# TravisWheelerLab/BATH

Measured on AMD Instinct MI355X. Metric: DP Gcells/s + residues/s through bathsearch pipeline at 1/2/4/8 MI355X, higher is better.
Workload: dtype u8/i16 integer scores (SSV: exact binary16), f32 Forward

## Files before the change

### bath_amd/csrc/bath_profile.hip

```cpp
#include <atomic>
#include <cctype>
#include <cmath>
#include <cstring>

#include "bath_common.hpp"
#include "host_model.hpp"

using namespace bath;

namespace bath {

static const double kLog2 = 0.69314718055994529;

double gumbel_surv(double x, double mu, double lambda) {
  double ey = -std::exp(-lambda * (x - mu));
  if (std::fabs(ey) < 5e-9) return -ey;
  return 1.0 - std::exp(ey);
}
double gumbel_invsurv(double p, double mu, double lambda) {
  double lp = (p < 5e-9) ? (std::pow(p, p) - 1) / p : std::log(-1. * std::log(1 - p));
  return mu - lp / lambda;
}
double exp_surv(double x, double mu, double lambda) { return (x < mu) ? 1.0 : std::exp(-lambda * (x - mu)); }

static inline uint8_t cost_u8(float scale, float sc) {
  float c = -1.0f * roundf(scale * sc);
  return (c > 255.) ? 255 : (uint8_t)(int)c;
}
static inline uint8_t cost_u8_biased(float scale, uint8_t bias, float sc) {
  float c = -1.0f * roundf(scale * sc);
  return (c > 255 - bias) ? 255 : (uint8_t)((int)c + bias);
}
static inline int16_t score_i16(float scale, float sc) {
  float v = roundf(scale * sc);
  if (v >= 32767.0) return 32767;
  if (v <= -32768.0) return -32768;
  return (int16_t)v;
}

void bias_filter_eo(const float *compo, float eo[kKp][2]) {
  for (int x = 0; x < 20; x++) { eo[x][0] = kAminoBg[x] / kAminoBg[x]; eo[x][1] = compo[x] / kAminoBg[x]; }
  for (int x : {20, 27, 28}) eo[x][0] = eo[x][1] = 1.0f;
  for (int x = 21; x <= 26; x++)
    for (int s = 0; s < 2; s++) {
      float num = 0.f, den = 0.f;
      for (int y = 0; y < 20; y++)
        if (amino_degen_has(x, y)) { num += (s == 0 ? kAminoBg[y] : compo[y]); den += kAminoBg[y]; }
      eo[x][s] = den > 0.f ? num / den : 0.f;
    }
}

template <class T>
static hipError_t upload(T **dst, const T *src, size_t n, hipStream_t st) {
  hipError_t e = hipMalloc((void **)dst, n * sizeof(T) + 64);
  if (e != hipSuccess) return e;
  return hipMemcpyAsync(*dst, src, n * sizeof(T), hipMemcpyHostToDevice, st);
}

int build_len_tables(const bath_hip_oprofile *om, int maxL) {
  std::lock_guard<std::mutex> lock(om->grow_mu);
  LenTables &lt = om->lt;
  if (maxL <= lt.maxL) return BATH_OK;
  bath_hip_ctx *ctx = om->ctx;
  int n = std::max(maxL, 4096) + 1;
  for (void *p : {(void *)lt.d_tjb, (void *)lt.d_xwmove, (void *)lt.d_pmove, (void *)lt.d_nullsc, (void *)lt.d_lt1, (void *)lt.d_lt2, (void *)lt.d_p1})
    if (p) om->retired.push_back(p);
  lt.d_tjb = nullptr; lt.d_xwmove = nullptr; lt.d_pmove = nullptr; lt.d_nullsc = nullptr; lt.d_lt1 = nullptr; lt.d_lt2 = nullptr; lt.d_p1 = nullptr;
  lt.h_tjb.resize(n); lt.h_xwmove.resize(n); lt.h_pmove.resize(n); lt.h_nullsc.resize(n);
  std::vector<float> lt1(n), lt2(n), p1v(n);
  for (int L = 0; L < n; L++) {
    lt.h_tjb[L] = cost_u8(om->scale_b, logf(3.0f / (float)(L + 3)));
    float pmove = (2.0f + om->nj) / ((float)L + 2.0f + om->nj);
    lt.h_pmove[L] = pmove;
    lt.h_xwmove[L] = score_i16(om->scale_w, logf(pmove));
    float p1 = (float)L / (float)(L + 1);
    p1v[L] = p1;
    lt.h_nullsc[L] = (float)((float)L * std::log((double)p1) + std::log(1. - p1));
    lt1[L] = (float)L * logf(p1);
    lt2[L] = logf((float)(1. - p1));
  }
  BATH_HIP_TRY(ctx, upload(&lt.d_tjb, lt.h_tjb.data(), n, ctx->stream));
  BATH_HIP_TRY(ctx, upload(&lt.d_xwmove, lt.h_xwmove.data(), n, ctx->stream));
  BATH_HIP_TRY(ctx, upload(&lt.d_pmove, lt.h_pmove.data(), n, ctx->stream));
  BATH_HIP_TRY(ctx, upload(&lt.d_nullsc, lt.h_nullsc.data(), n, ctx->stream));
  BATH_HIP_TRY(ctx, upload(&lt.d_lt1, lt1.data(), n, ctx->stream));
  BATH_HIP_TRY(ctx, upload(&lt.d_lt2, lt2.data(), n, ctx->stream));
  BATH_HIP_TRY(ctx, upload(&lt.d_p1, p1v.data(), n, ctx->stream));
  BATH_HIP_TRY(ctx, hipStreamSynchronize(ctx->stream));
  lt.maxL = n - 1;
  return BATH_OK;
}

}

int bath_hip_oprofile::ensure_len_tables(int maxL) const { return bath::build_len_tables(this, maxL); }


namespace bath { std::atomic<int> g_ctx_total{0}, g_ctx_internal{0}; }

extern "C" int bath_hip_init(int device, bath_hip_ctx **out) {
  *out = nullptr;
  int ndev = 0;
  if (hipGetDeviceCount(&ndev) != hipSuccess || ndev <= 0) return BATH_ENODEVICE;
  if (device < 0 || device >= ndev) return BATH_EINVAL;
  bath_hip_ctx *ctx = new bath_hip_ctx();
  ctx->device = device;
  if (const char *e = std::getenv("BATH_HIP_SYNC")) {
    static const bool once = [&] {
      (void)hipSetDevice(device);
      const unsigned fl = (e[0] == 'b') ? hipDeviceScheduleBlockingSync : (e[0] == 'y') ? hipDeviceScheduleYield : hipDeviceScheduleSpin;
      if (hipSetDeviceFlags(fl) != hipSuccess) (void)hipGetLastError();
      return true;
    }();
    (void)once;
  }
  if (hipSetDevice(device) != hipSuccess || hipGetDeviceProperties(&ctx->prop, device) != hipSuccess ||
      hipStreamCreateWithFlags(&ctx->stream, hipStreamNonBlocking) != hipSuccess) {
    delete ctx;
    return BATH_ENODEVICE;
  }
  bath::g_ctx_total.fetch_add(1);
  *out = ctx;
  return BATH_OK;
}

extern "C" void bath_hip_finalize(bath_hip_ctx *ctx) {
  if (!ctx) return;
  bath::g_ctx_total.fetch_sub(1);
  if (ctx->internal) bath::g_ctx_internal.fetch_sub(1);
  (void)hipSetDevice(ctx->device);
  (void)hipStreamSynchronize(ctx->stream);
  delete ctx->lane_pool; ctx->lane_pool = nullptr;
  for (bath_hip_ctx *lane : ctx->lanes) bath_hip_finalize(lane);
  ctx->lanes.clear();
  if (ctx->ev_lanes) (void)hipEventDestroy(ctx->ev_lanes);
  if (ctx->tail_stream) (void)hipStreamDestroy(ctx->tail_stream);
  if (ctx->aux) { bath_hip_finalize(ctx->aux); ctx->aux = nullptr; }
  if (ctx->aux2) { bath_hip_finalize(ctx->aux2); ctx->aux2 = nullptr; }
  if (ctx->aux3) { bath_hip_finalize(ctx->aux3); ctx->aux3 = nullptr; }
  for (auto &b : ctx->scratch) b.release();
  for (auto &b : ctx->pinned) b.release();
  for (auto &b : ctx->stage) b.release();
  ctx->results_pinned.release();
  for (auto e : ctx->ev_pool) (void)hipEventDestroy(e);
  for (auto e : ctx->span_events) (void)hipEventDestroy(e);
  if (ctx->ev_fork) (void)hipEventDestroy(ctx->ev_fork);
  if (ctx->ev_join) (void)hipEventDestroy(ctx->ev_join);
  if (ctx->copy_stream) (void)hipStreamDestroy(ctx->copy_stream);
  if (ctx->side_stream) (void)hipStreamDestroy(ctx->side_stream);
  (void)hipStreamDestroy(ctx->stream);
  delete ctx;
}

extern "C" int bath_hip_trim(bath_hip_ctx *ctx) {
  if (!ctx) return BATH_EINVAL;
  BATH_HIP_TRY(ctx, hipSetDevice(ctx->device));
  BATH_HIP_TRY(ctx, hipStreamSynchronize(ctx->stream));
  delete ctx->lane_pool; ctx->lane_pool = nullptr;
// ... 56 lines not shown
  if (!ctx) return BATH_EINVAL;
  ctx->fs_odds = on ? 1 : 0;
  for (bath_hip_ctx *l : ctx->lanes) l->fs_odds = ctx->fs_odds;
  return BATH_OK;
}

extern "C" int bath_hip_set_fs5_odds(bath_hip_ctx *ctx, int on) {
  if (!ctx) return BATH_EINVAL;
  ctx->fs5_odds = on ? 1 : 0;
  for (bath_hip_ctx *l : ctx->lanes) l->fs5_odds = ctx->fs5_odds;
  return BATH_OK;
}


extern "C" void bath_hip_oprofile_destroy(bath_hip_oprofile *om) {
  if (!om) return;
  for (void *p : {(void *)om->d_emit, (void *)om->d_ssv, (void *)om->d_msv, (void *)om->d_rb, (void *)om->d_rw, (void *)om->d_tw, (void *)om->d_rf, (void *)om->d_tf,
                  (void *)om->d_bias_eo, (void *)om->d_vit_rw, (void *)om->d_vit_tw2, (void *)om->d_vit_rank, (void *)om->lt.d_tjb, (void *)om->lt.d_xwmove, (void *)om->lt.d_pmove,
                  (void *)om->lt.d_nullsc, (void *)om->lt.d_lt1, (void *)om->lt.d_lt2, (void *)om->lt.d_p1, (void *)om->d_cons, (void *)om->d_msc, (void *)om->d_tsc, (void *)om->d_rfb, (void *)om->d_tfb})
    if (p) (void)hipFree(p);
  for (void *p : om->retired) (void)hipFree(p);
  delete om;
}

extern "C" int bath_hip_oprofile_set_consensus(bath_hip_oprofile *om, const char *consensus) {
  if (!om || !consensus) return BATH_EINVAL;
  bath_hip_ctx *ctx = om->ctx;
  static const char syms[] = "ACDEFGHIKLMNPQRSTVWY-BJZOUX*~";
  om->consensus.assign((size_t)om->M + 2, ' ');
  om->cons_digital.assign((size_t)om->M + 1, 255);
  for (int k = 1; k <= om->M && consensus[k]; k++) {
    om->consensus[(size_t)k] = consensus[k];
    const char *q = std::strchr(syms, std::toupper((unsigned char)consensus[k]));
    if (q) om->cons_digital[(size_t)k] = (uint8_t)(q - syms);
  }
  if (!om->d_cons) BATH_HIP_TRY(ctx, hipMalloc(&om->d_cons, (size_t)om->M + 1));
  BATH_HIP_TRY(ctx, hipMemcpy(om->d_cons, om->cons_digital.data(), (size_t)om->M + 1, hipMemcpyHostToDevice));
  return BATH_OK;
}

extern "C" int bath_hip_oprofile_M(const bath_hip_oprofile *om) { return om->M; }

extern "C" int bath_hip_oprofile_convert(bath_hip_ctx *ctx, const bath_profile *gm, bath_hip_oprofile **ret) {
  *ret = nullptr;
  const int M = gm->M;
  if (M < 1) { ctx->set_error("profile has no nodes"); return BATH_EINVAL; }
  const size_t W = (size_t)M + 1;
  auto msc = [&](int k, int x) { return gm->rsc[(size_t)x * W * 2 + 2 * k]; };
  auto tsc = [&](int k, int s) { return gm->tsc[(size_t)k * 8 + s]; };
  enum { MM, IM, DM, BM, MD, DD, MI, II };

  bath_hip_oprofile *om = new bath_hip_oprofile();
  { static std::atomic<uint64_t> next_uid{1}; om->uid = next_uid.fetch_add(1); }
  om->ctx = ctx; om->M = M; om->max_length = gm->max_length; om->nj = gm->nj; om->L0 = gm->L;
  std::memcpy(om->evparam, gm->evparam, sizeof om->evparam);
  std::memcpy(om->compo, gm->compo, sizeof om->compo);

  float maxsc = 0.0f;
  for (int x = 0; x < 20; x++)
    for (size_t i = 0; i < W * 2; i++) maxsc = std::max(maxsc, gm->rsc[(size_t)x * W * 2 + i]);
  om->scale_b = (float)(3.0 / kLog2);
  om->base_b = 190;
  om->bias_b = cost_u8(om->scale_b, (float)(-1.0 * maxsc));
  om->rb.assign((size_t)kKp * W, 255);
  for (int x = 0; x < kKp; x++)
    for (int k = 1; k <= M; k++) om->rb[x * W + k] = cost_u8_biased(om->scale_b, om->bias_b, msc(k, x));
  om->tbm_b = cost_u8(om->scale_b, logf(2.0f / ((float)M * (float)(M + 1))));
  om->tec_b = cost_u8(om->scale_b, logf(0.5f));

  om->scale_w = (float)(500.0 / kLog2);
  om->base_w = 12000;
  om->rw.assign((size_t)kKp * W, -32768);
  for (int x = 0; x < kKp; x++)
    for (int k = 1; k <= M; k++) om->rw[x * W + k] = score_i16(om->scale_w, msc(k, x));
  om->tw.assign(W * 8, -32768);
  for (int k = 1; k <= M; k++) {
    int16_t *t = &om->tw[(size_t)k * 8];
    for (int s : {BM, MM, IM, DM}) t[s] = std::min<int16_t>(score_i16(om->scale_w, tsc(k - 1, s)), 0);
    for (int s : {MD, MI}) t[s] = (k < M) ? std::min<int16_t>(score_i16(om->scale_w, tsc(k, s)), 0) : (int16_t)-32768;
    t[II] = (k < M) ? std::min<int16_t>(score_i16(om->scale_w, tsc(k, II)), -1) : (int16_t)-32768;
    t[DD] = (k < M) ? score_i16(om->scale_w, tsc(k, DD)) : (int16_t)-32768;
  }
  om->xw_E[0] = score_i16(om->scale_w, gm->xsc[0][0]);
  om->xw_E[1] = score_i16(om->scale_w, gm->xsc[0][1]);
  int ddb = -32768;
  for (int k = 2; k < M - 1; k++)
    ddb = std::max(ddb, (int)score_i16(om->scale_w, tsc(k, DD)) + (int)score_i16(om->scale_w, tsc(k + 1, DM)) -
                            (int)score_i16(om->scale_w, tsc(k + 1, BM)));
  om->ddbound_w = (int16_t)ddb;

  om->rf.assign((size_t)kKp * W, 0.f);
  for (int x = 0; x < kKp; x++)
    for (int k = 1; k <= M; k++) om->rf[x * W + k] = expf(msc(k, x));
  om->tf.assign(W * 8, 0.f);
  for (int k = 1; k <= M; k++) {
    float *t = &om->tf[(size_t)k * 8];
    for (int s : {BM, MM, IM, DM}) t[s] = expf(tsc(k - 1, s));
    for (int s : {MD, MI, II, DD}) t[s] = (k < M) ? expf(tsc(k, s)) : 0.f;
  }
  om->xf_E[0] = expf(gm->xsc[0][0]);
  om->xf_E[1] = expf(gm->xsc[0][1]);

  {
    std::vector<float> &pre = om->prefix_lengths, &suf = om->suffix_lengths;
    pre.assign(W, 0.f); suf.assign(W, 0.f);
    float total = 0;
    for (int k = 1; k < M; k++) {
      const float t_mi = om->tf[(size_t)k * 8 + MI], t_ii = om->tf[(size_t)k * 8 + II];
      pre[k] = (t_mi == 0) ? 1.f : (float)(1 + (int)(std::log(1e-7 / t_mi) / std::log((double)t_ii)));
      total += pre[k];
    }
    pre[0] = pre[M] = 0;
    for (int k = 1; k < M; k++) pre[k] /= total;
    suf[M] = pre[M - 1];
    for (int k = M - 1; k >= 1; k--) suf[k] = suf[k + 1] + pre[k - 1];
    for (int k = 2; k < M; k++) pre[k] += pre[k - 1];
  }

  static const bool wide = [] { const char *e = std::getenv("BATH_HIP_SSV_WIDE"); return e && e[0] == '1'; }();
  static const int g2max = [] { const char *e = std::getenv("BATH_HIP_SSV_G2_MAX"); return e ? std::atoi(e) : 304; }();
  int G = (!wide && M > 152 && M <= g2max) ? 2 : 1;
  while (G < 8 && M > 416 * G) G *= 2;
  if (M > 416 * G) { ctx->set_error("model longer than 3328 nodes"); delete om; return BATH_EINVAL; }
  int NR = ((M + G - 1) / G + 1) / 2;
  if (G == 1 && NR <= 112) NR = (NR + 3) / 4 * 4;
  else if (G == 2 && NR <= 76) NR = NR <= 40 ? 40 : (NR <= 72 ? (NR + 7) / 8 * 8 : 76);
  else NR = std::max((NR + 15) / 16 * 16, G > 1 ? 112 : 16);
  NR = std::max(NR, 16);
  om->NR = NR; om->G = G;
  om->ssv_row_bytes = 16 * ((NR * G / 4 + 1) | 1);
  {
    size_t rowsz = (size_t)om->ssv_row_bytes / 2;
    auto half_bits = [](float v) { const _Float16 h = (_Float16)v; int16_t b; std::memcpy(&b, &h, 2); return b; };
    std::vector<int16_t> tab((size_t)kSsvRows * rowsz, half_bits(-1.0f));
    for (int x = 0; x < kKp; x++)
      for (int k = 1; k <= M; k++) {
        const int g = (k - 1) / (2 * NR), q = (k - 1) - g * 2 * NR;
        const int cost = std::min((int)om->rb[x * W + k] - (int)om->bias_b, 127);
        tab[x * rowsz + (size_t)g * 2 * NR + 2 * (q % NR) + q / NR] = half_bits(-(float)cost / 2048.0f);
      }
    BATH_HIP_TRY(ctx, upload(&om->d_ssv, tab.data(), tab.size(), ctx->stream));
    if (G == 1 && NR <= 76) {
      std::vector<int16_t> mtab((size_t)kSsvRows * rowsz, half_bits(-1.0f));
      for (int x = 0; x < kKp; x++)
        for (int k = 1; k <= M; k++) {
          const int q = k - 1;
          const int inc = (int)om->bias_b - (int)om->rb[x * W + k];
          mtab[x * rowsz + 2 * (q % NR) + q / NR] = half_bits((float)inc / 2048.0f);
        }
      BATH_HIP_TRY(ctx, upload(&om->d_msv, mtab.data(), mtab.size(), ctx->stream));
    }
  }
  {
    int NRv = ((M + 1) / 2 + 15) / 16 * 16;
    if (NRv == 80) NRv = std::max(68, ((M + 1) / 2 + 3) / 4 * 4);
    if (NRv <= 112) {
      om->vit_NR = NRv;
      om->vit_rw_pitch = 4 * NRv + 16;
      const size_t rowsz = (size_t)om->vit_rw_pitch / 2;
      std::vector<int16_t> rwt((size_t)30 * rowsz, (int16_t)-32768);
      auto slot = [&](int node) { return node <= NRv ? 2 * (node - 1) : 2 * (node - NRv - 1) + 1; };
      for (int x = 0; x < kKp; x++)
        for (int k = 1; k <= M; k++) rwt[x * rowsz + slot(k)] = om->rw[x * W + k];
      std::vector<uint32_t> tw2((size_t)NRv * 8);
      std::vector<int16_t> rank((size_t)2 * NRv, (int16_t)32767);
      const int Q8 = std::max(2, ((M - 1) / 8) + 1);
      auto twv = [&](int node, int s) -> int { return node <= M ? (int)om->tw[(size_t)node * 8 + s] : -32768; };
      for (int r = 0; r < NRv; r++)
        for (int s = 0; s < 8; s++) tw2[(size_t)r * 8 + s] = ((uint32_t)(uint16_t)twv(r + 1, s)) | ((uint32_t)(uint16_t)twv(NRv + r + 1, s) << 16);
      for (int node = 1; node <= M; node++) rank[(size_t)slot(node)] = (int16_t)(((node - 1) % Q8) * 8 + (node - 1) / Q8);
      BATH_HIP_TRY(ctx, upload(&om->d_vit_rw, rwt.data(), rwt.size(), ctx->stream));
      BATH_HIP_TRY(ctx, upload(&om->d_vit_tw2, tw2.data(), tw2.size(), ctx->stream));
      BATH_HIP_TRY(ctx, upload(&om->d_vit_rank, rank.data(), rank.size(), ctx->stream));
    }
  }
  om->rb_stride = (int)W;
  BATH_HIP_TRY(ctx, upload(&om->d_rb, om->rb.data(), om->rb.size(), ctx->stream));
  BATH_HIP_TRY(ctx, upload(&om->d_rw, om->rw.data(), om->rw.size(), ctx->stream));
  BATH_HIP_TRY(ctx, upload(&om->d_tw, om->tw.data(), om->tw.size(), ctx->stream));
  BATH_HIP_TRY(ctx, upload(&om->d_rf, om->rf.data(), om->rf.size(), ctx->stream));
  BATH_HIP_TRY(ctx, upload(&om->d_tf, om->tf.data(), om->tf.size(), ctx->stream));
  {
    std::vector<float> tfb((size_t)(M + 2) * 8, 0.f), rfb((size_t)kKp * (M + 2), 0.f);
    std::memcpy(tfb.data(), om->tf.data(), sizeof(float) * (size_t)(M + 1) * 8);
    for (int x = 0; x < kKp; x++) std::memcpy(&rfb[(size_t)x * (M + 2)], &om->rf[(size_t)x * W], sizeof(float) * W);
    BATH_HIP_TRY(ctx, upload(&om->d_tfb, tfb.data(), tfb.size(), ctx->stream));
    BATH_HIP_TRY(ctx, upload(&om->d_rfb, rfb.data(), rfb.size(), ctx->stream));
    BATH_HIP_TRY(ctx, hipStreamSynchronize(ctx->stream));
  }
  {
    std::vector<float> lm((size_t)kKp * W, -INFINITY);
    for (int x = 0; x < kKp; x++)
      for (int k = 1; k <= M; k++) lm[(size_t)x * W + k] = msc(k, x);
    BATH_HIP_TRY(ctx, upload(&om->d_msc, lm.data(), lm.size(), ctx->stream));
    BATH_HIP_TRY(ctx, upload(&om->d_tsc, gm->tsc, (size_t)M * 8, ctx->stream));
    BATH_HIP_TRY(ctx, hipStreamSynchronize(ctx->stream));
  }
  {
    float eo[kKp][2];
    bias_filter_eo(om->compo, eo);
    BATH_HIP_TRY(ctx, upload(&om->d_bias_eo, &eo[0][0], (size_t)kKp * 2, ctx->stream));
  }
  BATH_HIP_TRY(ctx, hipStreamSynchronize(ctx->stream));
  int st = om->ensure_len_tables(4096);
  if (st != BATH_OK) { bath_hip_oprofile_destroy(om); return st; }
  *ret = om;
  return BATH_OK;
}

extern "C" int bath_hip_oprofile_scalars(const bath_hip_oprofile *om, int L, bath_oprofile_scalars *o) {
  int st = om->ensure_len_tables(L);
  if (st != BATH_OK) return st;
  o->tbm_b = om->tbm_b; o->tec_b = om->tec_b; o->tjb_b = om->lt.h_tjb[L]; o->base_b = om->base_b; o->bias_b = om->bias_b;
  o->scale_b = om->scale_b;
  o->xw[0][0] = om->xw_E[0]; o->xw[0][1] = om->xw_E[1];
  for (int s = 1; s < 4; s++) { o->xw[s][0] = 0; o->xw[s][1] = om->lt.h_xwmove[L]; }
  o->scale_w = om->scale_w; o->base_w = om->base_w; o->ddbound_w = om->ddbound_w;
  o->xf[0][0] = om->xf_E[0]; o->xf[0][1] = om->xf_E[1];
  for (int s = 1; s < 4; s++) { o->xf[s][1] = om->lt.h_pmove[L]; o->xf[s][0] = 1.0f - om->lt.h_pmove[L]; }
  return BATH_OK;
}

extern "C" int bath_hip_oprofile_get_ssv_scores(const bath_hip_oprofile *om, uint8_t *arr) {
  const size_t W = (size_t)om->M + 1;
  std::memset(arr, 0, W * kKp);
  for (int k = 1; k <= om->M; k++)
    for (int x = 0; x < kKp; x++) arr[(size_t)k * kKp + x] = om->rb[x * W + k];
  return BATH_OK;
}
extern "C" int bath_hip_oprofile_get_vit(const bath_hip_oprofile *om, int16_t *rw, int16_t *tw) {
  std::memcpy(rw, om->rw.data(), om->rw.size() * sizeof(int16_t));
  std::memcpy(tw, om->tw.data(), om->tw.size() * sizeof(int16_t));
  return BATH_OK;
}
extern "C" int bath_hip_oprofile_get_fwd(const bath_hip_oprofile *om, float *rf, float *tf) {
  std::memcpy(rf, om->rf.data(), om->rf.size() * sizeof(float));
  std::memcpy(tf, om->tf.data(), om->tf.size() * sizeof(float));
  return BATH_OK;
}


extern "C" void bath_hip_seqs_destroy(bath_hip_seqs *sq) {
  if (!sq) return;
  for (bath_hip_seqs *part : sq->parts) bath_hip_seqs_destroy(part);
  sq->parts.clear();
  if (sq->is_part) { sq->d_data = nullptr; sq->d_len = nullptr; sq->d_context = nullptr; }
  for (void *p : {(void *)sq->d_data, (void *)sq->d_off, (void *)sq->d_len, (void *)sq->d_context, (void *)sq->d_tile_desc, (void *)sq->d_tile_first,
                  (void *)sq->d_packed, (void *)sq->d_poff, sq->d_exc})
    if (p) (void)hipFree(p);
  if (sq->ev_upload) (void)hipEventDestroy(sq->ev_upload);
  delete sq;
}

extern "C" int64_t bath_hip_seqs_count(const bath_hip_seqs *sq) { return sq->n; }

extern "C" int bath_hip_seqs_set_context(bath_hip_seqs *sq, const int32_t *context) {
  if (!sq || sq->is_part) return BATH_EINVAL;
  bath_hip_ctx *ctx = sq->ctx;
  for (bath_hip_seqs *part : sq->parts) bath_hip_seqs_destroy(part);
  sq->parts.clear();
  sq->cache_minlen = -1;
  if (!context) { if (sq->d_context) (void)hipFree(sq->d_context); sq->d_context = nullptr; sq->h_context.clear(); return BATH_OK; }
  for (int64_t i = 0; i < sq->n; i++) if (context[i] < 0 || context[i] > sq->h_len[(size_t)i]) { ctx->set_error("context longer than its window"); return BATH_EINVAL; }
  sq->h_context.assign(context, context + sq->n);
  if (!sq->d_context) BATH_HIP_TRY(ctx, hipMalloc((void **)&sq->d_context, (size_t)std::max<int64_t>(sq->n, 1) * sizeof(int32_t)));
  if (sq->n > 0) BATH_HIP_TRY(ctx, hipMemcpy(sq->d_context, sq->h_context.data(), (size_t)sq->n * sizeof(int32_t), hipMemcpyHostToDevice));
  return BATH_OK;
}

extern "C" int bath_hip_seqs_create(bath_hip_ctx *ctx, const uint8_t *dsq, const int64_t *offsets, int64_t n, bath_hip_seqs **ret) {
  *ret = nullptr;
  if (n < 0) return BATH_EINVAL;
  bath_hip_seqs *sq = new bath_hip_seqs();
  sq->ctx = ctx; sq->n = n;
  sq->h_off.resize(n); sq->h_len.resize(n);
  int64_t pos = 0;
  bool contiguous_ok = true;
  for (int64_t i = 0; i < n; i++) {
    int64_t L = offsets[i + 1] - offsets[i];
    if (L < 0 || L > INT32_MAX) { delete sq; ctx->set_error("bad sequence offsets"); return BATH_EINVAL; }
    sq->h_off[i] = pos; sq->h_len[i] = (int32_t)L;
    if (pos != offsets[i] - offsets[0]) contiguous_ok = false;
    sq->maxlen = std::max(sq->maxlen, (int32_t)L);
    sq->total += L;
    pos += (L + 15) / 16 * 16;
  }
  sq->total_aligned = pos;
  size_t bytes = (size_t)pos + 64;
  BATH_HIP_TRY(ctx, hipMalloc((void **)&sq->d_data, bytes));
  BATH_HIP_TRY(ctx, hipMalloc((void **)&sq->d_off, (size_t)std::max<int64_t>(n, 1) * sizeof(int64_t)));
  BATH_HIP_TRY(ctx, hipMalloc((void **)&sq->d_len, (size_t)std::max<int64_t>(n, 1) * sizeof(int32_t)));
  BATH_HIP_TRY(ctx, hipMemsetAsync(sq->d_data, 0x1d, bytes, ctx->stream));
  std::vector<uint8_t> staged;
  if (n > 0) {
    if (contiguous_ok) {
      BATH_HIP_TRY(ctx, hipMemcpyAsync(sq->d_data, dsq + offsets[0], (size_t)(offsets[n] - offsets[0]), hipMemcpyHostToDevice, ctx->stream));
    } else {
      staged.assign((size_t)pos, 0x1d);
      for (int64_t i = 0; i < n; i++) std::memcpy(staged.data() + sq->h_off[i], dsq + offsets[i], (size_t)sq->h_len[i]);
      BATH_HIP_TRY(ctx, hipMemcpyAsync(sq->d_data, staged.data(), staged.size(), hipMemcpyHostToDevice, ctx->stream));
    }
    BATH_HIP_TRY(ctx, hipMemcpyAsync(sq->d_off, sq->h_off.data(), (size_t)n * sizeof(int64_t), hipMemcpyHostToDevice, ctx->stream));
    BATH_HIP_TRY(ctx, hipMemcpyAsync(sq->d_len, sq->h_len.data(), (size_t)n * sizeof(int32_t), hipMemcpyHostToDevice, ctx->stream));
  }
  BATH_HIP_TRY(ctx, hipStreamSynchronize(ctx->stream));
  *ret = sq;
  return BATH_OK;
}


namespace {
struct ExcRec { int64_t seq; int32_t pos, code; };

__global__ __launch_bounds__(256) void unpack2_kernel(const uint8_t *__restrict__ packed, const int64_t *__restrict__ poff, const int64_t *__restrict__ off,
                                                      const int32_t *__restrict__ len, uint8_t *__restrict__ data, int64_t n) {
  const int64_t s = (int64_t)blockIdx.x * 4 + (threadIdx.x >> 6);
  if (s >= n) return;
  const int lane = threadIdx.x & 63;
  const int L = len[s];
  const int nb = (L + 3) >> 2;
  const uint8_t *src = packed + poff[s];
  uint8_t *dst = data + off[s];
  const int j_lo = blockIdx.y * 4096, j_hi = min((nb + 3) >> 2, j_lo + 4096);
// ... 97 lines not shown
```

### bath_amd/csrc/bath_viterbi.hip

```cpp
#include <algorithm>

#include "bath_common.hpp"
#include "bath_kernels.hpp"
#include "bath_launch.hpp"

using namespace bath;

namespace bath {

__device__ __forceinline__ s16x2 pk_adds(s16x2 a, s16x2 b) { return __builtin_elementwise_add_sat(a, b); }
__device__ __forceinline__ s16x2 pk_max(s16x2 a, s16x2 b) { return __builtin_elementwise_max(a, b); }
__device__ __forceinline__ s16x2 as_s2(unsigned v) { return __builtin_bit_cast(s16x2, v); }
__device__ __forceinline__ unsigned as_u(s16x2 v) { return __builtin_bit_cast(unsigned, v); }

struct VitLaneTables {
  const int16_t *rw;
  int rw_pitch_bytes;
  const uint32_t *tw2;
  const int16_t *rank;
};

struct VitLaneConsts {
  int M, base_w, xwE_loop, xwE_move, Q8;
  float scale_w;
  double invP_vit, invP_msv;
  float scale_b;
  int base_b, tec_b, bias_b;
};

typedef uint32_t u32x16 __attribute__((ext_vector_type(16)));

template <int NR>
#ifndef BATH_VIT_WAVES
#define BATH_VIT_WAVES 1
#endif
__global__ __launch_bounds__(256, (NR <= 76 ? BATH_VIT_WAVES : 1)) void vit_lane_kernel(SeqView sq, VitLaneTables tb, const uint32_t *__restrict__ tw2g, VitLaneConsts c, const int16_t *__restrict__ xwmove_tab,
                                                          const uint8_t *__restrict__ tjb_tab, const int32_t *__restrict__ todo, int64_t ntodo,
                                                          const int *__restrict__ ntodo_dev, const int *__restrict__ skip_dev, float *__restrict__ sc, int32_t *__restrict__ status,
                                                          const float *__restrict__ filtersc, const uint8_t *__restrict__ ssv_scores,
                                                          WindowRec *__restrict__ wins, int *__restrict__ win_count, int win_cap, int32_t *__restrict__ kminmax) {
  extern __shared__ __attribute__((aligned(16))) char lds[];
  char *s_rw = lds;
  int16_t *s_rank = reinterpret_cast<int16_t *>(lds + 30 * tb.rw_pitch_bytes);
  {
    const uint32_t *src = reinterpret_cast<const uint32_t *>(tb.rw);
    uint32_t *dst = reinterpret_cast<uint32_t *>(s_rw);
    for (int i = threadIdx.x; i < 30 * tb.rw_pitch_bytes / 4; i += blockDim.x) dst[i] = src[i];
    for (int i = threadIdx.x; i < 2 * NR; i += blockDim.x) s_rank[i] = tb.rank[i];
  }
  __syncthreads();
  if (ntodo_dev) ntodo = *ntodo_dev;
  const int64_t t = (int64_t)blockIdx.x * blockDim.x + threadIdx.x + (skip_dev ? *skip_dev : 0);
  if (t - (threadIdx.x & 63) >= ntodo) return;
  const bool live = t < ntodo;
  const int64_t sid = live ? (todo ? (int64_t)todo[t] : t) : (todo ? (int64_t)todo[0] : 0);
  const int L = live ? sq.len[sid] : 0;
  const uint8_t *s = sq.data + sq.off[sid];
  const int Lw = wave_max_i32(L);
  const bool do_win = (wins != nullptr);
  const int M = c.M;

  const int xw_move = xwmove_tab[L];
  int sc_thresh = 0, sc_ext_thresh = 0, skip_until = 0, kmin = 1 << 30, kmax = 0;
  if (do_win && live) {
    const double fsc = (double)filtersc[sid];
    sc_thresh = (int)(int16_t)(int)ceil(((fsc + 0.69314718055994529 * c.invP_vit + 3.0) * (double)c.scale_w) -
                                        (double)(float)c.xwE_move - (double)(float)xw_move + (double)(float)c.base_w);
    sc_ext_thresh = (int)ceil(((fsc + 0.69314718055994529 * c.invP_msv + 3.0) * (double)c.scale_b) + c.base_b + c.tec_b + (int)tjb_tab[L]);
  }
  const s16x2 NEG = {-32768, -32768};
  s16x2 Mr[NR], Ir[NR], Dr[NR];
#pragma unroll
  for (int r = 0; r < NR; r++) Mr[r] = Ir[r] = Dr[r] = NEG;
  int xN = c.base_w;
  int xB = (int16_t)(xN + xw_move);
  int xJ = -32768, xC = -32768;
  bool overflow = false;
  short ePrev = -32768;

  uint32_t wnext = (0 < L) ? *reinterpret_cast<const uint32_t *>(s) : 0x1d1d1d1du;
  for (int i0 = 0; i0 < Lw; i0 += 4) {
    const uint32_t w = wnext;
    wnext = (i0 + 4 < L) ? *reinterpret_cast<const uint32_t *>(s + i0 + 4) : 0x1d1d1d1du;
#pragma unroll 1
    for (int j = 0; j < 4; j++) {
      const int i = i0 + j + 1;
      const bool on = (i <= L) && !overflow;
      int x = (w >> (8 * j)) & 0xff;
      x = (i <= L) ? min(x, kKp - 1) : 29;
      const char *rowbase = s_rw + x * tb.rw_pitch_bytes;
      const s16x2 xBv = {(short)xB, (short)xB};
      s16x2 xEv = NEG;
      unsigned pM = (as_u(Mr[NR - 1]) << 16) | 0x8000u, pI = (as_u(Ir[NR - 1]) << 16) | 0x8000u, pD = (as_u(Dr[NR - 1]) << 16) | 0x8000u;
      s16x2 dpk = NEG;
      s16x2 cpk = {(short)-32768, ePrev};
      int twz = 0;
      asm volatile("" : "+s"(twz));
      const uint32_t *tw = tw2g + twz;
      u32x16 t_c, t_n;
      int4 e_c = *reinterpret_cast<const int4 *>(rowbase), e_n = e_c;
      asm volatile("s_load_dwordx16 %0, %1, 0x0" : "=s"(t_c) : "s"(tw));
#pragma unroll
      for (int r = 0; r < NR; r += 2) {
        asm volatile("s_waitcnt lgkmcnt(0)" ::: "memory");
        __builtin_amdgcn_sched_barrier(0);
        if ((r & 3) == 0 && r + 4 < NR) e_n = *reinterpret_cast<const int4 *>(rowbase + 4 * (r + 4));
        if (r + 2 < NR) asm volatile("s_load_dwordx16 %0, %1, %2" : "=s"(t_n) : "s"(tw), "i"((r + 2) * 32));
        __builtin_amdgcn_sched_barrier(0);
        const unsigned em[2] = {(r & 3) ? (unsigned)e_c.z : (unsigned)e_c.x, (r & 3) ? (unsigned)e_c.w : (unsigned)e_c.y};
#pragma unroll
        for (int q = 0; q < 2; q++) {
          const int rr = r + q;
          const unsigned tMM = t_c[8 * q + 0], tIM = t_c[8 * q + 1], tDM = t_c[8 * q + 2], tBM = t_c[8 * q + 3];
          const unsigned tMD = t_c[8 * q + 4], tDD = t_c[8 * q + 5], tMI = t_c[8 * q + 6], tII = t_c[8 * q + 7];
          const unsigned oM = as_u(Mr[rr]), oI = as_u(Ir[rr]);
          const unsigned oD = as_u(pk_max(Dr[rr], cpk));
          cpk = pk_adds(cpk, as_s2(tDD));
          const s16x2 ms = as_s2(pM), is = as_s2(pI), ds = as_s2(pD);
          s16x2 sv = pk_adds(xBv, as_s2(tBM));
          sv = pk_max(sv, pk_adds(ms, as_s2(tMM)));
          sv = pk_max(sv, pk_adds(is, as_s2(tIM)));
          sv = pk_max(sv, pk_adds(ds, as_s2(tDM)));
          sv = pk_adds(sv, as_s2(em[q]));
          Ir[rr] = pk_max(pk_adds(as_s2(oM), as_s2(tMI)), pk_adds(as_s2(oI), as_s2(tII)));
          const s16x2 dcv = pk_adds(sv, as_s2(tMD));
          xEv = pk_max(xEv, sv);
          Mr[rr] = sv;
          Dr[rr] = dpk;
          dpk = pk_max(dcv, pk_adds(dpk, as_s2(tDD)));
          pM = oM; pI = oI; pD = oD;
        }
        if (r + 2 < NR) t_c = t_n;
        if ((r & 3) == 2 && r + 2 < NR) e_c = e_n;
        asm volatile("" : "+v"(Mr[r]), "+v"(Mr[r + 1]), "+v"(Ir[r]), "+v"(Ir[r + 1]), "+v"(Dr[r]), "+v"(Dr[r + 1]), "+v"(dpk), "+v"(cpk), "+v"(xEv));
        __builtin_amdgcn_sched_barrier(0);
      }
      ePrev = dpk.x;
      if (on) {
        const int xE = max((int)xEv.x, (int)xEv.y);
        if (xE >= 32767) overflow = true;
        else {
          xN = (int16_t)(xN + 0);
          xC = (int16_t)max(xC + 0, xE + c.xwE_move);
          xJ = (int16_t)max(xJ + 0, xE + c.xwE_loop);
          xB = (int16_t)max(xJ + xw_move, xN + xw_move);
          if (do_win && i > skip_until && xE >= sc_thresh) {
            int rank = 32767;
#pragma unroll
            for (int r = 0; r < NR; r++) {
              if ((int)Mr[r].x == xE) rank = min(rank, (int)s_rank[2 * r]);
              if ((int)Mr[r].y == xE) rank = min(rank, (int)s_rank[2 * r + 1]);
            }
            const int k_start = (rank / 8) + c.Q8 * (rank % 8) + 1;
            int max_k_end = k_start, max_i_end = i, sc_ext = sc_ext_thresh, max_sc_ext = sc_ext, since = 0;
            int kk = k_start + 1, nn = i + 1;
            while (kk <= M && nn <= L) {
              sc_ext += c.bias_b - (int)ssv_scores[(size_t)kk * kKp + min((int)s[nn - 1], kKp - 1)];
              if (sc_ext >= max_sc_ext) { max_sc_ext = sc_ext; max_k_end = kk; max_i_end = nn; since = 0; }
              else if (++since == 5) break;
              kk++; nn++;
            }
            const int slot = atomicAdd(win_count, 1);
            if (slot < win_cap) wins[slot] = WindowRec{(int32_t)sid, i, max_k_end, max_k_end - k_start + 1, 0.0f};
            kmax = max(kmax, max_k_end);
            kmin = min(kmin, k_start);
            skip_until = max_i_end;
          }
        }
      }
    }
  }
  if (live) {
    if (overflow) { sc[sid] = INFINITY; status[sid] = BATH_ERANGE; }
    else if (xC > -32768) {
      float r = (float)xC + (float)xw_move - (float)c.base_w;
      r /= c.scale_w;
      r = (float)((double)r - 3.0);
      sc[sid] = r; status[sid] = BATH_OK;
    } else { sc[sid] = -INFINITY; status[sid] = BATH_OK; }
    if (do_win && kminmax) { kminmax[2 * sid] = kmin; kminmax[2 * sid + 1] = kmax; }
  }
}

constexpr int kLenBins = 2048;
__device__ __forceinline__ void len_block_range(int n, int &lo, int &hi) {
  const int per = (n + (int)gridDim.x - 1) / (int)gridDim.x;
  lo = min(n, (int)blockIdx.x * per); hi = min(n, lo + per);
}
__global__ __launch_bounds__(256) void len_hist_kernel(const int32_t *__restrict__ todo, const int *__restrict__ ntodo_dev, const int32_t *__restrict__ len,
                                                       int *__restrict__ hist) {
  __shared__ int s_cnt[kLenBins];
  for (int i = threadIdx.x; i < kLenBins; i += blockDim.x) s_cnt[i] = 0;
  __syncthreads();
  int lo, hi;
  len_block_range(*ntodo_dev, lo, hi);
  for (int j = lo + threadIdx.x; j < hi; j += blockDim.x) atomicAdd(&s_cnt[min(len[todo[j]], kLenBins - 1)], 1);
  __syncthreads();
  for (int i = threadIdx.x; i < kLenBins; i += blockDim.x) if (s_cnt[i]) atomicAdd(&hist[i], s_cnt[i]);
}
__global__ void len_scan_kernel(int *__restrict__ hist ) {
  __shared__ int tmp[kLenBins];
  for (int i = threadIdx.x; i < kLenBins; i += blockDim.x) tmp[i] = hist[i];
  __syncthreads();
  if (threadIdx.x == 0) {
    int run = 0;
    for (int b = kLenBins - 1; b >= 0; b--) { const int cnt = tmp[b]; tmp[b] = run; run += cnt; }
  }
  __syncthreads();
  for (int i = threadIdx.x; i < kLenBins; i += blockDim.x) hist[i] = tmp[i];
}
__global__ __launch_bounds__(256) void len_scatter_kernel(const int32_t *__restrict__ todo, const int *__restrict__ ntodo_dev, const int32_t *__restrict__ len,
                                                          int *__restrict__ cursor, int32_t *__restrict__ sorted) {
  __shared__ int s_cnt[kLenBins];
  for (int i = threadIdx.x; i < kLenBins; i += blockDim.x) s_cnt[i] = 0;
  __syncthreads();
  int lo, hi;
  len_block_range(*ntodo_dev, lo, hi);
  for (int j = lo + threadIdx.x; j < hi; j += blockDim.x) atomicAdd(&s_cnt[min(len[todo[j]], kLenBins - 1)], 1);
  __syncthreads();
  for (int i = threadIdx.x; i < kLenBins; i += blockDim.x) { const int c = s_cnt[i]; if (c) s_cnt[i] = atomicAdd(&cursor[i], c); }
  __syncthreads();
  for (int j = lo + threadIdx.x; j < hi; j += blockDim.x) {
    const int cnd = todo[j];
    sorted[atomicAdd(&s_cnt[min(len[cnd], kLenBins - 1)], 1)] = cnd;
  }
}

int vit_lane_supported(const bath_hip_oprofile *om) { return om->vit_NR > 0; }

const int *len_sort_count_longer(const int *d_bins, int T) { return d_bins + std::min(T + 1, kLenBins - 1); }

int launch_len_sort(bath_hip_ctx *ctx, const int32_t *d_todo, const int *d_ntodo, const int32_t *d_len, int *d_bins, int32_t *d_sorted) {
  BATH_HIP_TRY(ctx, hipMemsetAsync(d_bins, 0, kLenBins * sizeof(int), ctx->stream));
  hipLaunchKernelGGL(len_hist_kernel, dim3(256), dim3(256), 0, ctx->stream, d_todo, d_ntodo, d_len, d_bins);
  hipLaunchKernelGGL(len_scan_kernel, dim3(1), dim3(256), 0, ctx->stream, d_bins);
  hipLaunchKernelGGL(len_scatter_kernel, dim3(256), dim3(256), 0, ctx->stream, d_todo, d_ntodo, d_len, d_bins, d_sorted);
  BATH_HIP_TRY(ctx, hipGetLastError());
  return BATH_OK;
}

int launch_vit_lane(bath_hip_ctx *ctx, const bath_hip_oprofile *om, SeqView v, const int32_t *d_todo, int64_t ntodo, const int *ntodo_dev,
                    float *d_sc, int32_t *d_status, const VitWindowArgs *wa, const int *skip_dev) {
  if (ntodo == 0) return BATH_OK;
  VitLaneTables tb{om->d_vit_rw, om->vit_rw_pitch, om->d_vit_tw2, om->d_vit_rank};
  VitLaneConsts c{};
  c.M = om->M; c.base_w = om->base_w; c.xwE_loop = om->xw_E[0]; c.xwE_move = om->xw_E[1]; c.Q8 = std::max(2, ((om->M - 1) / 8) + 1);
  c.scale_w = om->scale_w; c.scale_b = om->scale_b; c.base_b = om->base_b; c.tec_b = om->tec_b; c.bias_b = om->bias_b;
  const float *fsc = nullptr; const uint8_t *ssv = nullptr; WindowRec *wins = nullptr; int *wc = nullptr; int cap = 0; int32_t *kmm = nullptr;
  if (wa) { c.invP_vit = wa->invP_vit; c.invP_msv = wa->invP_msv; fsc = wa->d_filtersc; ssv = wa->d_ssv_scores; wins = (WindowRec *)wa->d_wins; wc = wa->d_win_count; cap = wa->win_cap; kmm = wa->d_kminmax; }
  const int NRv = om->vit_NR;
  const size_t shmem = (size_t)30 * om->vit_rw_pitch + (size_t)2 * NRv * 2 + 16;
  const int blocks = (int)((ntodo + 255) / 256);
  bool launched = false;
#define BATH_VITL_CASE(N)                                                                                                              \
  if (!launched && NRv == N) {                                                                                                         \
    hipLaunchKernelGGL(vit_lane_kernel<N>, dim3(blocks), dim3(256), shmem, ctx->stream, v, tb, tb.tw2, c, om->lt.d_xwmove, om->lt.d_tjb, d_todo, ntodo, \
                       ntodo_dev, skip_dev, d_sc, d_status, fsc, ssv, wins, wc, cap, kmm);                                                       \
    launched = true;                                                                                                                   \
  }
  BATH_VITL_CASE(16) BATH_VITL_CASE(32) BATH_VITL_CASE(48) BATH_VITL_CASE(64) BATH_VITL_CASE(68) BATH_VITL_CASE(72) BATH_VITL_CASE(76) BATH_VITL_CASE(80)
  BATH_VITL_CASE(96) BATH_VITL_CASE(112)
#undef BATH_VITL_CASE
  if (!launched) { ctx->set_error("lane-per-target Viterbi kernel: unsupported model length"); return BATH_EINVAL; }
  BATH_HIP_TRY(ctx, hipGetLastError());
  return BATH_OK;
}

}
```

Before: 196.1 billion.

## Drop per-row D array from Viterbi lane kernel and allow two waves for NR up to 80

The Viterbi lane kernel no longer keeps a register array Dr[NR] for the previous row's delete states. Delete values are instead carried through a running dold term plus a small link (dNR, dNR1) between rows, and the row update is moved into a shared host/device helper header. The launch-bounds occupancy hint now defaults to two waves per SIMD for NR up to 80, where before it was one unless a macro was set. Fewer live VGPRs should let more waves hide latency, but the recomputed delete chain changes the dependency structure and could add instructions or spills.

```diff
diff --git a/bath_amd/csrc/bath_profile.hip b/bath_amd/csrc/bath_profile.hip
--- a/bath_amd/csrc/bath_profile.hip
+++ b/bath_amd/csrc/bath_profile.hip
@@ -4,6 +4,7 @@
 #include <cstring>
 
 #include "bath_common.hpp"
+#include "bath_vit_rows.hpp"
 #include "host_model.hpp"
 
 using namespace bath;
@@ -366,23 +367,14 @@
     }
   }
   {
-    int NRv = ((M + 1) / 2 + 15) / 16 * 16;
-    if (NRv == 80) NRv = std::max(68, ((M + 1) / 2 + 3) / 4 * 4);
-    if (NRv <= 112) {
+    const int NRv = vit_lane_pairs(M);
+    if (NRv > 0) {
       om->vit_NR = NRv;
-      om->vit_rw_pitch = 4 * NRv + 16;
-      const size_t rowsz = (size_t)om->vit_rw_pitch / 2;
-      std::vector<int16_t> rwt((size_t)30 * rowsz, (int16_t)-32768);
-      auto slot = [&](int node) { return node <= NRv ? 2 * (node - 1) : 2 * (node - NRv - 1) + 1; };
-      for (int x = 0; x < kKp; x++)
-        for (int k = 1; k <= M; k++) rwt[x * rowsz + slot(k)] = om->rw[x * W + k];
+      om->vit_rw_pitch = vit_lane_row_pitch(NRv);
+      std::vector<int16_t> rwt((size_t)30 * om->vit_rw_pitch / 2);
       std::vector<uint32_t> tw2((size_t)NRv * 8);
-      std::vector<int16_t> rank((size_t)2 * NRv, (int16_t)32767);
-      const int Q8 = std::max(2, ((M - 1) / 8) + 1);
-      auto twv = [&](int node, int s) -> int { return node <= M ? (int)om->tw[(size_t)node * 8 + s] : -32768; };
-      for (int r = 0; r < NRv; r++)
-        for (int s = 0; s < 8; s++) tw2[(size_t)r * 8 + s] = ((uint32_t)(uint16_t)twv(r + 1, s)) | ((uint32_t)(uint16_t)twv(NRv + r + 1, s) << 16);
-      for (int node = 1; node <= M; node++) rank[(size_t)slot(node)] = (int16_t)(((node - 1) % Q8) * 8 + (node - 1) / Q8);
+      std::vector<int16_t> rank((size_t)2 * NRv);
+      vit_lane_tables(M, kKp, om->rw.data(), om->tw.data(), NRv, rwt.data(), tw2.data(), rank.data());
       BATH_HIP_TRY(ctx, upload(&om->d_vit_rw, rwt.data(), rwt.size(), ctx->stream));
       BATH_HIP_TRY(ctx, upload(&om->d_vit_tw2, tw2.data(), tw2.size(), ctx->stream));
       BATH_HIP_TRY(ctx, upload(&om->d_vit_rank, rank.data(), rank.size(), ctx->stream));
diff --git a/bath_amd/csrc/bath_vit_rows.hpp b/bath_amd/csrc/bath_vit_rows.hpp
--- /dev/null
+++ b/bath_amd/csrc/bath_vit_rows.hpp
@@ -0,0 +1,152 @@
+#pragma once
+#include <cmath>
+#include <cstdint>
+
+#if defined(__HIPCC__)
+#define BATH_VIT_FN __host__ __device__ __forceinline__
+#else
+#define BATH_VIT_FN inline
+#endif
+
+namespace bath {
+
+struct VitPairHost {
+  struct T { int16_t x, y; };
+  static int16_t sat(int v) { return (int16_t)(v > 32767 ? 32767 : (v < -32768 ? -32768 : v)); }
+  static T adds(T a, T b) { return T{sat((int)a.x + b.x), sat((int)a.y + b.y)}; }
+  static T max(T a, T b) { return T{a.x > b.x ? a.x : b.x, a.y > b.y ? a.y : b.y}; }
+  static T from_bits(unsigned v) { return T{(int16_t)(uint16_t)(v & 0xffffu), (int16_t)(uint16_t)(v >> 16)}; }
+  static unsigned bits(T v) { return (unsigned)(uint16_t)v.x | ((unsigned)(uint16_t)v.y << 16); }
+  static int lo(T v) { return v.x; }
+  static int hi(T v) { return v.y; }
+};
+
+enum { VIT_MM = 0, VIT_IM, VIT_DM, VIT_BM, VIT_MD, VIT_DD, VIT_MI, VIT_II };
+
+struct VitRowLink {
+  int dNR = -32768;
+  int dNR1 = -32768;
+};
+
+template <class P>
+struct VitRowPass {
+  typedef typename P::T T;
+  unsigned pM, pI, pD;
+  T dold;
+  T cpk;
+  T dpk, dlast;
+  T xEv, xBv;
+
+  BATH_VIT_FN void begin(T MrLast, T IrLast, const VitRowLink &prev, int xB) {
+    pM = (P::bits(MrLast) << 16) | 0x8000u;
+    pI = (P::bits(IrLast) << 16) | 0x8000u;
+    pD = ((unsigned)(uint16_t)prev.dNR << 16) | 0x8000u;
+    const T neg = P::from_bits(0x80008000u);
+    dold = dpk = dlast = xEv = neg;
+    cpk = P::from_bits(0x8000u | ((unsigned)(uint16_t)prev.dNR1 << 16));
+    xBv = P::from_bits((unsigned)(uint16_t)xB * 0x10001u);
+  }
+
+  template <class TW>
+  BATH_VIT_FN void step(T &Mr, T &Ir, const TW &t, int tbase, unsigned em) {
+    const T tMM = P::from_bits(t[tbase + VIT_MM]), tIM = P::from_bits(t[tbase + VIT_IM]), tDM = P::from_bits(t[tbase + VIT_DM]), tBM = P::from_bits(t[tbase + VIT_BM]);
+    const T tMD = P::from_bits(t[tbase + VIT_MD]), tDD = P::from_bits(t[tbase + VIT_DD]), tMI = P::from_bits(t[tbase + VIT_MI]), tII = P::from_bits(t[tbase + VIT_II]);
+    const T oMv = Mr, oIv = Ir;
+    const unsigned oM = P::bits(oMv), oI = P::bits(oIv);
+    const unsigned oD = P::bits(P::max(dold, cpk));
+    cpk = P::adds(cpk, tDD);
+    dold = P::max(P::adds(oMv, tMD), P::adds(dold, tDD));
+    T sv = P::adds(xBv, tBM);
+    sv = P::max(sv, P::adds(P::from_bits(pM), tMM));
+    sv = P::max(sv, P::adds(P::from_bits(pI), tIM));
+    sv = P::max(sv, P::adds(P::from_bits(pD), tDM));
+    sv = P::adds(sv, P::from_bits(em));
+    Ir = P::max(P::adds(oMv, tMI), P::adds(oIv, tII));
+    const T dcv = P::adds(sv, tMD);
+    xEv = P::max(xEv, sv);
+    Mr = sv;
+    dlast = dpk;
+    dpk = P::max(dcv, P::adds(dpk, tDD));
+    pM = oM; pI = oI; pD = oD;
+  }
+
+  BATH_VIT_FN int xE() const { return P::lo(xEv) > P::hi(xEv) ? P::lo(xEv) : P::hi(xEv); }
+  BATH_VIT_FN VitRowLink link() const { VitRowLink l; l.dNR = P::lo(dlast); l.dNR1 = P::lo(dpk); return l; }
+};
+
+struct VitSpecials {
+  int xN, xB, xJ, xC;
+  BATH_VIT_FN void begin(int base_w, int xw_move) { xN = base_w; xB = (int16_t)(xN + xw_move); xJ = -32768; xC = -32768; }
+  BATH_VIT_FN bool row(int xE, int xwE_move, int xwE_loop, int xw_move) {
+    if (xE >= 32767) return false;
+    xN = (int16_t)(xN + 0);
+    xC = (int16_t)(xC + 0 > xE + xwE_move ? xC + 0 : xE + xwE_move);
+    xJ = (int16_t)(xJ + 0 > xE + xwE_loop ? xJ + 0 : xE + xwE_loop);
+    xB = (int16_t)(xJ + xw_move > xN + xw_move ? xJ + xw_move : xN + xw_move);
+    return true;
+  }
+};
+
+struct VitWindow { int k_start, max_k_end, max_i_end; };
+
+struct VitWinThresh { int sc, sc_ext; };
+BATH_VIT_FN VitWinThresh vit_window_thresholds(double fsc, double invP_vit, double invP_msv, float scale_w, float scale_b, int xwE_move, int xw_move, int base_w,
+                                               int base_b, int tec_b, int tjb) {
+  VitWinThresh t;
+  t.sc = (int)(int16_t)(int)ceil(((fsc + 0.69314718055994529 * invP_vit + 3.0) * (double)scale_w) - (double)(float)xwE_move - (double)(float)xw_move + (double)(float)base_w);
+  t.sc_ext = (int)ceil(((fsc + 0.69314718055994529 * invP_msv + 3.0) * (double)scale_b) + base_b + tec_b + tjb);
+  return t;
+}
+
+template <class P, int NR>
+BATH_VIT_FN int vit_window_rank(const typename P::T (&Mr)[NR], const int16_t *rank, int xE) {
+  int best = 32767;
+#pragma unroll
+  for (int r = 0; r < NR; r++) {
+    if (P::lo(Mr[r]) == xE) best = best < (int)rank[2 * r] ? best : (int)rank[2 * r];
+    if (P::hi(Mr[r]) == xE) best = best < (int)rank[2 * r + 1] ? best : (int)rank[2 * r + 1];
+  }
+  return best;
+}
+
+BATH_VIT_FN VitWindow vit_window_extend(int rank, int Q8, int i, int M, int L, const uint8_t *s , const uint8_t *ssv_scores, int Kp,
+                                        int bias_b, int sc_ext_thresh) {
+  VitWindow w;
+  w.k_start = (rank / 8) + Q8 * (rank % 8) + 1;
+  w.max_k_end = w.k_start; w.max_i_end = i;
+  int sc_ext = sc_ext_thresh, max_sc_ext = sc_ext, since = 0;
+  int kk = w.k_start + 1, nn = i + 1;
+  while (kk <= M && nn <= L) {
+    const int x = (int)s[nn - 1] < Kp - 1 ? (int)s[nn - 1] : Kp - 1;
+    sc_ext += bias_b - (int)ssv_scores[(size_t)kk * Kp + x];
+    if (sc_ext >= max_sc_ext) { max_sc_ext = sc_ext; w.max_k_end = kk; w.max_i_end = nn; since = 0; }
+    else if (++since == 5) break;
+    kk++; nn++;
+  }
+  return w;
+}
+
+
+inline int vit_lane_pairs(int M) {
+  int NRv = ((M + 1) / 2 + 15) / 16 * 16;
+  if (NRv == 80) { NRv = ((M + 1) / 2 + 3) / 4 * 4; if (NRv < 68) NRv = 68; }
+  return NRv <= 112 ? NRv : 0;
+}
+inline int vit_lane_row_pitch(int NRv) { return 4 * NRv + 16; }
+inline int vit_lane_q8(int M) { const int q = ((M - 1) / 8) + 1; return q > 2 ? q : 2; }
+
+inline void vit_lane_tables(int M, int Kp, const int16_t *rw, const int16_t *tw, int NRv, int16_t *rwt, uint32_t *tw2, int16_t *rank) {
+  const size_t W = (size_t)M + 1, rowsz = (size_t)vit_lane_row_pitch(NRv) / 2;
+  for (size_t z = 0; z < 30 * rowsz; z++) rwt[z] = (int16_t)-32768;
+  for (int z = 0; z < 2 * NRv; z++) rank[z] = (int16_t)32767;
+  auto slot = [&](int node) { return node <= NRv ? 2 * (node - 1) : 2 * (node - NRv - 1) + 1; };
+  for (int x = 0; x < Kp; x++)
+    for (int k = 1; k <= M; k++) rwt[x * rowsz + slot(k)] = rw[x * W + k];
+  auto twv = [&](int node, int s) -> int { return node <= M ? (int)tw[(size_t)node * 8 + s] : -32768; };
+  for (int r = 0; r < NRv; r++)
+    for (int s = 0; s < 8; s++) tw2[(size_t)r * 8 + s] = ((uint32_t)(uint16_t)twv(r + 1, s)) | ((uint32_t)(uint16_t)twv(NRv + r + 1, s) << 16);
+  const int Q8 = vit_lane_q8(M);
+  for (int node = 1; node <= M; node++) rank[(size_t)slot(node)] = (int16_t)(((node - 1) % Q8) * 8 + (node - 1) / Q8);
+}
+
+}
diff --git a/bath_amd/csrc/bath_viterbi.hip b/bath_amd/csrc/bath_viterbi.hip
--- a/bath_amd/csrc/bath_viterbi.hip
+++ b/bath_amd/csrc/bath_viterbi.hip
@@ -3,6 +3,7 @@
 #include "bath_common.hpp"
 #include "bath_kernels.hpp"
 #include "bath_launch.hpp"
+#include "bath_vit_rows.hpp"
 
 using namespace bath;
 
@@ -30,11 +31,21 @@
 
 typedef uint32_t u32x16 __attribute__((ext_vector_type(16)));
 
+struct VitPair {
+  typedef s16x2 T;
+  static __device__ __forceinline__ T adds(T a, T b) { return pk_adds(a, b); }
+  static __device__ __forceinline__ T max(T a, T b) { return pk_max(a, b); }
+  static __device__ __forceinline__ T from_bits(unsigned v) { return as_s2(v); }
+  static __device__ __forceinline__ unsigned bits(T v) { return as_u(v); }
+  static __device__ __forceinline__ int lo(T v) { return v.x; }
+  static __device__ __forceinline__ int hi(T v) { return v.y; }
+};
+
+constexpr int kVitTwoWavesMaxNR = 80;
+constexpr int vit_lane_waves(int NR) { return NR <= kVitTwoWavesMaxNR ? 2 : 1; }
+
 template <int NR>
-#ifndef BATH_VIT_WAVES
-#define BATH_VIT_WAVES 1
-#endif
-__global__ __launch_bounds__(256, (NR <= 76 ? BATH_VIT_WAVES : 1)) void vit_lane_kernel(SeqView sq, VitLaneTables tb, const uint32_t *__restrict__ tw2g, VitLaneConsts c, const int16_t *__restrict__ xwmove_tab,
+__global__ __launch_bounds__(256, vit_lane_waves(NR)) void vit_lane_kernel(SeqView sq, VitLaneTables tb, const uint32_t *__restrict__ tw2g, VitLaneConsts c, const int16_t *__restrict__ xwmove_tab,
                                                           const uint8_t *__restrict__ tjb_tab, const int32_t *__restrict__ todo, int64_t ntodo,
                                                           const int *__restrict__ ntodo_dev, const int *__restrict__ skip_dev, float *__restrict__ sc, int32_t *__restrict__ status,
                                                           const float *__restrict__ filtersc, const uint8_t *__restrict__ ssv_scores,
@@ -63,20 +74,18 @@
   const int xw_move = xwmove_tab[L];
   int sc_thresh = 0, sc_ext_thresh = 0, skip_until = 0, kmin = 1 << 30, kmax = 0;
   if (do_win && live) {
-    const double fsc = (double)filtersc[sid];
-    sc_thresh = (int)(int16_t)(int)ceil(((fsc + 0.69314718055994529 * c.invP_vit + 3.0) * (double)c.scale_w) -
-                                        (double)(float)c.xwE_move - (double)(float)xw_move + (double)(float)c.base_w);
-    sc_ext_thresh = (int)ceil(((fsc + 0.69314718055994529 * c.invP_msv + 3.0) * (double)c.scale_b) + c.base_b + c.tec_b + (int)tjb_tab[L]);
+    const VitWinThresh th = vit_window_thresholds((double)filtersc[sid], c.invP_vit, c.invP_msv, c.scale_w, c.scale_b, c.xwE_move, xw_move, c.base_w,
+                                                  c.base_b, c.tec_b, (int)tjb_tab[L]);
+    sc_thresh = th.sc; sc_ext_thresh = th.sc_ext;
   }
   const s16x2 NEG = {-32768, -32768};
-  s16x2 Mr[NR], Ir[NR], Dr[NR];
+  s16x2 Mr[NR], Ir[NR];
 #pragma unroll
-  for (int r = 0; r < NR; r++) Mr[r] = Ir[r] = Dr[r] = NEG;
-  int xN = c.base_w;
-  int xB = (int16_t)(xN + xw_move);
-  int xJ = -32768, xC = -32768;
+  for (int r = 0; r < NR; r++) Mr[r] = Ir[r] = NEG;
+  VitSpecials sp;
+  sp.begin(c.base_w, xw_move);
   bool overflow = false;
-  short ePrev = -32768;
+  VitRowLink link;
 
   uint32_t wnext = (0 < L) ? *reinterpret_cast<const uint32_t *>(s) : 0x1d1d1d1du;
   for (int i0 = 0; i0 < Lw; i0 += 4) {
@@ -89,11 +98,8 @@
       int x = (w >> (8 * j)) & 0xff;
       x = (i <= L) ? min(x, kKp - 1) : 29;
       const char *rowbase = s_rw + x * tb.rw_pitch_bytes;
-      const s16x2 xBv = {(short)xB, (short)xB};
-      s16x2 xEv = NEG;
-      unsigned pM = (as_u(Mr[NR - 1]) << 16) | 0x8000u, pI = (as_u(Ir[NR - 1]) << 16) | 0x8000u, pD = (as_u(Dr[NR - 1]) << 16) | 0x8000u;
-      s16x2 dpk = NEG;
-      s16x2 cpk = {(short)-32768, ePrev};
+      VitRowPass<VitPair> row;
+      row.begin(Mr[NR - 1], Ir[NR - 1], link, sp.xB);
       int twz = 0;
       asm volatile("" : "+s"(twz));
       const uint32_t *tw = tw2g + twz;
@@ -109,67 +115,29 @@
         __builtin_amdgcn_sched_barrier(0);
         const unsigned em[2] = {(r & 3) ? (unsigned)e_c.z : (unsigned)e_c.x, (r & 3) ? (unsigned)e_c.w : (unsigned)e_c.y};
 #pragma unroll
-        for (int q = 0; q < 2; q++) {
-          const int rr = r + q;
-          const unsigned tMM = t_c[8 * q + 0], tIM = t_c[8 * q + 1], tDM = t_c[8 * q + 2], tBM = t_c[8 * q + 3];
-          const unsigned tMD = t_c[8 * q + 4], tDD = t_c[8 * q + 5], tMI = t_c[8 * q + 6], tII = t_c[8 * q + 7];
-          const unsigned oM = as_u(Mr[rr]), oI = as_u(Ir[rr]);
-          const unsigned oD = as_u(pk_max(Dr[rr], cpk));
-          cpk = pk_adds(cpk, as_s2(tDD));
-          const s16x2 ms = as_s2(pM), is = as_s2(pI), ds = as_s2(pD);
-          s16x2 sv = pk_adds(xBv, as_s2(tBM));
-          sv = pk_max(sv, pk_adds(ms, as_s2(tMM)));
-          sv = pk_max(sv, pk_adds(is, as_s2(tIM)));
-          sv = pk_max(sv, pk_adds(ds, as_s2(tDM)));
-          sv = pk_adds(sv, as_s2(em[q]));
-          Ir[rr] = pk_max(pk_adds(as_s2(oM), as_s2(tMI)), pk_adds(as_s2(oI), as_s2(tII)));
-          const s16x2 dcv = pk_adds(sv, as_s2(tMD));
-          xEv = pk_max(xEv, sv);
-          Mr[rr] = sv;
-          Dr[rr] = dpk;
-          dpk = pk_max(dcv, pk_adds(dpk, as_s2(tDD)));
-          pM = oM; pI = oI; pD = oD;
-        }
+        for (int q = 0; q < 2; q++) row.step(Mr[r + q], Ir[r + q], t_c, 8 * q, em[q]);
         if (r + 2 < NR) t_c = t_n;
         if ((r & 3) == 2 && r + 2 < NR) e_c = e_n;
-        asm volatile("" : "+v"(Mr[r]), "+v"(Mr[r + 1]), "+v"(Ir[r]), "+v"(Ir[r + 1]), "+v"(Dr[r]), "+v"(Dr[r + 1]), "+v"(dpk), "+v"(cpk), "+v"(xEv));
+        asm volatile("" : "+v"(Mr[r]), "+v"(Mr[r + 1]), "+v"(Ir[r]), "+v"(Ir[r + 1]), "+v"(row.dold), "+v"(row.dpk), "+v"(row.cpk), "+v"(row.xEv));
         __builtin_amdgcn_sched_barrier(0);
       }
-      ePrev = dpk.x;
+      link = row.link();
       if (on) {
-        const int xE = max((int)xEv.x, (int)xEv.y);
-        if (xE >= 32767) overflow = true;
-        else {
-          xN = (int16_t)(xN + 0);
-          xC = (int16_t)max(xC + 0, xE + c.xwE_move);
-          xJ = (int16_t)max(xJ + 0, xE + c.xwE_loop);
-          xB = (int16_t)max(xJ + xw_move, xN + xw_move);
-          if (do_win && i > skip_until && xE >= sc_thresh) {
-            int rank = 32767;
-#pragma unroll
-            for (int r = 0; r < NR; r++) {
-              if ((int)Mr[r].x == xE) rank = min(rank, (int)s_rank[2 * r]);
-              if ((int)Mr[r].y == xE) rank = min(rank, (int)s_rank[2 * r + 1]);
-            }
-            const int k_start = (rank / 8) + c.Q8 * (rank % 8) + 1;
-            int max_k_end = k_start, max_i_end = i, sc_ext = sc_ext_thresh, max_sc_ext = sc_ext, since = 0;
-            int kk = k_start + 1, nn = i + 1;
-            while (kk <= M && nn <= L) {
-              sc_ext += c.bias_b - (int)ssv_scores[(size_t)kk * kKp + min((int)s[nn - 1], kKp - 1)];
-              if (sc_ext >= max_sc_ext) { max_sc_ext = sc_ext; max_k_end = kk; max_i_end = nn; since = 0; }
-              else if (++since == 5) break;
-              kk++; nn++;
-            }
-            const int slot = atomicAdd(win_count, 1);
-            if (slot < win_cap) wins[slot] = WindowRec{(int32_t)sid, i, max_k_end, max_k_end - k_start + 1, 0.0f};
-            kmax = max(kmax, max_k_end);
-            kmin = min(kmin, k_start);
-            skip_until = max_i_end;
-          }
+        const int xE = row.xE();
+        if (!sp.row(xE, c.xwE_move, c.xwE_loop, xw_move)) overflow = true;
+        else if (do_win && i > skip_until && xE >= sc_thresh) {
+          const int rank = vit_window_rank<VitPair, NR>(Mr, s_rank, xE);
+          const VitWindow vw = vit_window_extend(rank, c.Q8, i, M, L, s, ssv_scores, kKp, c.bias_b, sc_ext_thresh);
+          const int slot = atomicAdd(win_count, 1);
+          if (slot < win_cap) wins[slot] = WindowRec{(int32_t)sid, i, vw.max_k_end, vw.max_k_end - vw.k_start + 1, 0.0f};
+          kmax = max(kmax, vw.max_k_end);
+          kmin = min(kmin, vw.k_start);
+          skip_until = vw.max_i_end;
         }
       }
     }
   }
+  const int xC = sp.xC;
   if (live) {
     if (overflow) { sc[sid] = INFINITY; status[sid] = BATH_ERANGE; }
     else if (xC > -32768) {
```

Result: no change. 196.4 billion, median of 3 (+0.1%).
